# coecms/xmhw

Measured on AMD Instinct MI355X. Metric: grid-cells/sec for threshold() on 40yr daily SST, higher is better.
Workload: dtype f32 in / f64 out; 1 GPU; 0.25deg global (configs[2]): 1036800 cells per step, 1982-2021 (T=14610), windowHalfWidth=5, pctile=90, smoothPercentileWidth=31, nan_frac=0.0, skipna=False; cells_rank0=1036800, T=14610, D=366, kernel=clim_sorted_f32 (sorted row-lists in LDS, 2 lanes per cell, layout 40), slabs=1, gather=none

## Files before the change

include/xmhw_amd.h:

```cpp
#ifndef XMHW_AMD_H
#define XMHW_AMD_H

#include <stddef.h>
#include <stdint.h>

#ifdef __cplusplus
extern "C" {
#endif

#define XMHW_OK 0
#define XMHW_ERR_INVALID 1
#define XMHW_ERR_HIP 2
#define XMHW_ERR_UNSUPPORTED 3
#define XMHW_ERR_NOMEM 4
#define XMHW_ERR_COMM 5

#define XMHW_KERNEL_AUTO 0
#define XMHW_KERNEL_RING 1
#define XMHW_KERNEL_GENERIC 2

int xmhw_version(void);
const char *xmhw_arch(void);
const char *xmhw_last_error(void);
int xmhw_device_count(int *count);
// ... 29 lines not shown
                   void *dst_host);
int xmhw_pad_gaps(void *ts_dev, int itemsize, int64_t T, int64_t C, int64_t ld, const double *x_dev,
                  double max_gap, void *stream);
int xmhw_stream_create(void **stream);
int xmhw_stream_destroy(void *stream);
int xmhw_stream_sync(void *stream);
int xmhw_event_create(void **event);
int xmhw_stream_wait_event(void *stream, void *event);
int xmhw_event_destroy(void *event);
int xmhw_event_record(void *event, void *stream);
int xmhw_event_elapsed_ms(void *start, void *stop, float *ms);

typedef struct xmhw_plan xmhw_plan;

int xmhw_plan_create(const int32_t *doy_host, int64_t T, int32_t window_half_width,
                     xmhw_plan **plan);
int xmhw_plan_destroy(xmhw_plan *plan);
int xmhw_plan_info(const xmhw_plan *plan, int32_t *D, int32_t *ntracks,
                   int32_t *kernel, int32_t *nsteps, int32_t *step_min);
int xmhw_plan_doys(const xmhw_plan *plan, int32_t *doys_out );
int xmhw_plan_set_kernel(xmhw_plan *plan, int32_t kernel);
int xmhw_plan_set_narrowing(xmhw_plan *plan, int32_t enable);
int xmhw_plan_set_timing(xmhw_plan *plan, int32_t enable);
int xmhw_plan_kernel_ms(xmhw_plan *plan, int32_t calls_back, float *ms);
int xmhw_plan_narrowed(xmhw_plan *plan, int32_t *narrowed_out);
int xmhw_plan_set_chunks(xmhw_plan *plan, int32_t nchunks);
int xmhw_plan_chunks_in_use(const xmhw_plan *plan, int64_t C, int32_t *nchunks);
int xmhw_plan_table(const xmhw_plan *plan, int32_t years_per_lane, uint32_t *table_out,
                    int32_t *ntracks_padded);
int xmhw_plan_sorted_info(const xmhw_plan *plan, int64_t C, int32_t *keys_per_list, int32_t *lds_bytes_per_wave,
                          int32_t *pieces);
int xmhw_plan_sorted_table(const xmhw_plan *plan, int32_t pieces, int32_t *nchunks, int32_t *nrows, int32_t *ntp,
                           int32_t *chunks_out, uint32_t *table_out, uint32_t *flags_out);

int xmhw_debug_stats_available(void);
int xmhw_plan_debug_stats_n(xmhw_plan *plan, int enable, uint64_t *out, int32_t n);
int xmhw_plan_debug_stats(xmhw_plan *plan, int enable, uint64_t *out8);

enum {
    XMHW_LAYOUT_AUTO = -2,
    XMHW_LAYOUT_RING1 = -1,
    XMHW_LAYOUT_RING2_8LANE = 8,
    XMHW_LAYOUT_RING2_4LANE = 10,
    XMHW_LAYOUT_RING2_16LANE = 12,
    XMHW_LAYOUT_RING3_8LANE = 20,
    XMHW_LAYOUT_RING3_4LANE = 21,
    XMHW_LAYOUT_RING3_2LANE = 22,
    XMHW_LAYOUT_SORTED = 40
};
int xmhw_plan_set_layout(xmhw_plan *plan, int32_t layout);
int xmhw_plan_layout_in_use(const xmhw_plan *plan, int32_t *layout);
int xmhw_sorted_device_ok(int32_t *holds);
int xmhw_plan_set_ring2(xmhw_plan *plan, int32_t variant);
int xmhw_plan_ring2_in_use(const xmhw_plan *plan, int32_t *variant);
int xmhw_plan_f64_mode(const xmhw_plan *plan, int32_t *variant);

int xmhw_clim_raw_f32(xmhw_plan *plan, const float *ts_dev, int64_t C, int64_t ld,
                      double q, int negate, double *thresh_dev, double *seas_dev,
                      int64_t ldo, void *stream);
int xmhw_clim_raw_f64(xmhw_plan *plan, const double *ts_dev, int64_t C, int64_t ld,
                      double q, int negate, double *thresh_dev, double *seas_dev,
                      int64_t ldo, void *stream);
int xmhw_clim_raw_i16(xmhw_plan *plan, const int16_t *codes_dev, int64_t C, int64_t ld, int big_endian,
                      int has_scale, double scale_factor, double add_offset, int has_fill, int32_t fill_code,
                      int decoded_itemsize, double q, int negate, double *thresh_dev, double *seas_dev,
                      int64_t ldo, void *stream);
// ... 268 lines not shown
```

xmhw_amd/csrc/capi.cpp:

```cpp
#include "../../include/xmhw_amd.h"

#include <hip/hip_runtime.h>
#include <unistd.h>

#include <cerrno>
#include <cmath>

#include <algorithm>
#include <cstdio>
#include <cstdlib>
#include <atomic>
#include <cstring>
#include <map>
#include <memory>
#include <mutex>
#include <new>
#include <string>
#include <type_traits>
#include <vector>

#include "kernels.h"
#include "plan.h"

namespace {

thread_local std::string g_err;

int fail(int code, const std::string& msg) {
    g_err = msg;
    return code;
}
int hip_fail(hipError_t e, const char* what) {
    if (e == hipErrorOutOfMemory) {
        (void)hipGetLastError();
        return fail(XMHW_ERR_NOMEM, std::string(what) + ": out of device memory");
    }
    return fail(XMHW_ERR_HIP, std::string(what) + ": " + hipGetErrorString(e));
}
}
int xmhw_set_error_(int code, const std::string& msg) { return fail(code, msg); }
namespace {
#define HIP_TRY(expr)                                        \
    do {                                                     \
        hipError_t _e = (expr);                              \
        if (_e != hipSuccess) return hip_fail(_e, #expr);    \
    } while (0)

constexpr int kSubs = 8;
constexpr double kSortedMinQ = 0.85;
inline bool sorted_serves(double q) { return q >= kSortedMinQ || q <= 1.0 - kSortedMinQ; }

}

struct xmhw_plan {
    xmhw::Plan host;
    std::mutex mu;
    bool uploaded = false;
    int32_t yps = 0;
    int32_t subs = 0;
    int32_t nchunks = 0;
    uint32_t* d_table = nullptr;
    int32_t yps2 = 0;
    int32_t subs2 = 0;
    int32_t ring2_variant = -2;
    uint32_t* d_table2 = nullptr;
    uint32_t* d_sflags = nullptr;
    int32_t yps64 = 0;
    uint32_t* d_table64 = nullptr;
    xmhw::DevChunk* d_chunks = nullptr;
    int32_t* d_row_ptr = nullptr;
    int32_t* d_centres = nullptr;
    unsigned long long* d_stats = nullptr;
    uint32_t* d_tablex = nullptr;
    int32_t ypsx = 0, subsx = 0;
    uint32_t* d_narrow_flag = nullptr;
    bool narrowing = true;
    int32_t yps_s = 0;
    uint32_t* d_table_s = nullptr;
    xmhw::DevSortedChunk* d_chunks_s = nullptr;
    uint32_t* d_sflags_s = nullptr;
    xmhw::DevChunk* d_chunks_i = nullptr;
    int32_t nchunks_s = 0, nchunks_i = 0;
    int64_t sorted_pieces = -1;
    int32_t sorted_built = 0;
    bool timing = false;
    hipEvent_t tev[32] = {};
    uint64_t tcalls = 0;

    ~xmhw_plan() {
        if (d_stats) (void)hipFree(d_stats);
        for (hipEvent_t e : tev) if (e) (void)hipEventDestroy(e);
        if (d_table_s) (void)hipFree(d_table_s);
        if (d_chunks_s) (void)hipFree(d_chunks_s);
        if (d_sflags_s) (void)hipFree(d_sflags_s);
        if (d_chunks_i) (void)hipFree(d_chunks_i);
        if (d_narrow_flag) (void)hipFree(d_narrow_flag);
        if (d_tablex) (void)hipFree(d_tablex);
        if (d_table) (void)hipFree(d_table);
        if (d_table64) (void)hipFree(d_table64);
        if (d_table2) (void)hipFree(d_table2);
        if (d_sflags) (void)hipFree(d_sflags);
        if (d_chunks) (void)hipFree(d_chunks);
        if (d_row_ptr) (void)hipFree(d_row_ptr);
        if (d_centres) (void)hipFree(d_centres);
    }
};

namespace {

int32_t ring2_resolved(const xmhw_plan* p);
int32_t ring2_legacy(const xmhw_plan* p);

struct X64Choice { int32_t variant = -1, yps = 0; };
X64Choice x64_choice(const xmhw_plan* p) {
    static const bool on = [] { const char* v = std::getenv("XMHW_RING2_F64"); return !(v && v[0] == '0'); }();
    X64Choice c;
    if (!on || p->ring2_variant == -1) return c;
    const int32_t y8 = xmhw::ring2_pick_yps(p->host.w, p->host.ntracks, 8);
    static const bool lds_on = [] { const char* v = std::getenv("XMHW_RING2_F64_LDS"); return !(v && v[0] == '0'); }();
    static const bool r3_on = [] { const char* v = std::getenv("XMHW_RING3_F64"); return !(v && v[0] == '0'); }();
    static const bool r3_4 = [] { const char* v = std::getenv("XMHW_RING3_F64_LANES"); return !(v && v[0] == '8'); }();
    if (r3_on && r3_4) {
        const int32_t y4 = xmhw::ring3_pick_yps(p->host.w, p->host.ntracks, 4);
        if (y4 > 0 && xmhw::ring3_x64_supported(p->host.w, y4, 4)) {
            c.variant = 21;
            c.yps = y4;
            return c;
        }
    }
    if (r3_on && y8 > 0 && xmhw::ring3_pick_yps(p->host.w, p->host.ntracks, 8) == y8 &&
        xmhw::ring3_x64_supported(p->host.w, y8, 8)) {
        c.variant = 20;
        c.yps = y8;
        return c;
    }
    if (y8 > 0 && (y8 <= 4 || lds_on) && xmhw::ring2_x64_supported(p->host.w, y8, 8)) {
        c.variant = 8;
        c.yps = y8;
        return c;
    }
    const int32_t y16 = xmhw::ring2_pick_yps(p->host.w, p->host.ntracks, 12);
    if (y16 > 0 && y16 <= 6 && xmhw::ring2_x64_supported(p->host.w, y16, 12)) {
        c.variant = 12;
        c.yps = y16;
// ... 88 lines not shown
    static std::mutex mu;
    static int state[64];
    static bool init = false;
    std::lock_guard<std::mutex> lock(mu);
    if (!init) { for (int& v : state) v = -1; init = true; }
    int dev = 0;
    if (hipGetDevice(&dev) != hipSuccess || dev < 0 || dev >= 64) return 0;
    if (state[dev] >= 0) return state[dev];
    uint32_t* d_bad = nullptr;
    uint32_t bad = 1;
    if (hipMalloc(&d_bad, sizeof(uint32_t)) != hipSuccess) return 0;
    const bool ran = xmhw::sorted_lds_probe(d_bad, nullptr) == hipSuccess &&
                     hipMemcpy(&bad, d_bad, sizeof(uint32_t), hipMemcpyDeviceToHost) == hipSuccess;
    (void)hipFree(d_bad);
    if (!ran) return 0;
    state[dev] = bad == 0 ? 1 : 0;
    return state[dev];
}

int upload_sorted(xmhw_plan* p, int64_t C) {
    const xmhw::Plan& h = p->host;
    if (!sorted_usable(p) || sorted_device_ok() != 1) { p->nchunks_s = 0; return XMHW_OK; }
    const int32_t yps = xmhw::sorted_pick_yps(h.w, h.ntracks);
    const int64_t waves = (C + 31) / 32;
    const int64_t pieces = h.nchunks_req > 0 ? h.nchunks_req : (1536 + waves - 1) / std::max<int64_t>(waves, 1);
    if (!p->d_table_s || p->yps_s != yps || p->sorted_pieces != pieces) {
        HIP_TRY(hipDeviceSynchronize());
        for (void** q : {reinterpret_cast<void**>(&p->d_table_s), reinterpret_cast<void**>(&p->d_sflags_s),
                         reinterpret_cast<void**>(&p->d_chunks_s), reinterpret_cast<void**>(&p->d_chunks_i)})
            if (*q) { HIP_TRY(hipFree(*q)); *q = nullptr; }
        const xmhw::Plan::SortedPlan sp = h.sorted_plan(2 * yps, 24, pieces);
        p->sorted_built = 0;
        p->nchunks_i = 0;
        if (!sp.chunks.empty()) {
            std::vector<xmhw::DevSortedChunk> cs(sp.chunks.size());
            for (size_t i = 0; i < cs.size(); ++i) cs[i] = {sp.chunks[i].warm_start, sp.chunks[i].begin, sp.chunks[i].end, sp.chunks[i].trow0};
            std::stable_sort(cs.begin(), cs.end(), [](const xmhw::DevSortedChunk& a, const xmhw::DevSortedChunk& b) {
                return a.end - a.warm_start > b.end - b.warm_start;
            });
            HIP_TRY(hipMalloc(&p->d_table_s, sizeof(uint32_t) * sp.table.size()));
            HIP_TRY(hipMemcpy(p->d_table_s, sp.table.data(), sizeof(uint32_t) * sp.table.size(), hipMemcpyHostToDevice));
            HIP_TRY(hipMalloc(&p->d_sflags_s, sizeof(uint32_t) * sp.flags.size()));
            HIP_TRY(hipMemcpy(p->d_sflags_s, sp.flags.data(), sizeof(uint32_t) * sp.flags.size(), hipMemcpyHostToDevice));
            HIP_TRY(hipMalloc(&p->d_chunks_s, sizeof(xmhw::DevSortedChunk) * cs.size()));
            HIP_TRY(hipMemcpy(p->d_chunks_s, cs.data(), sizeof(xmhw::DevSortedChunk) * cs.size(), hipMemcpyHostToDevice));
            p->sorted_built = static_cast<int32_t>(cs.size());
        }
        p->yps_s = yps;
        p->sorted_pieces = pieces;
    }
    p->nchunks_s = p->sorted_built;
    return XMHW_OK;
}

int upload(xmhw_plan* p, int64_t C) {
    std::lock_guard<std::mutex> lock(p->mu);
    {
        const int rc = upload_sorted(p, C);
        if (rc != XMHW_OK) return rc;
    }
    const int32_t nchunks = auto_chunks(p, C);
    const X64Choice xc0 = x64_choice(p);
    const int32_t xsubs0 = xc0.variant == 21 ? 4 : 8;
    const bool need_x = (xc0.variant == 8 || xc0.variant == 20 || xc0.variant == 21) &&
                        !(p->subs2 == xsubs0 && p->yps2 == xc0.yps);
    if (p->uploaded && nchunks == p->nchunks &&
        p->subs2 == xmhw::ring2_subs(ring2_resolved(p)) &&
        p->yps2 == (ring2_resolved(p) >= 0 ? xmhw::ring2_pick_yps(p->host.w, p->host.ntracks, ring2_resolved(p)) : 0) &&
        (!need_x || (p->ypsx == xc0.yps && p->subsx == xsubs0)))
        return XMHW_OK;
    const xmhw::Plan& h = p->host;
    if (!p->uploaded) {
// ... 63 lines not shown
template <typename T>
int clim_raw(xmhw_plan* plan, const T* ts, int64_t C, int64_t ld, double q, int negate,
             double* thresh, double* seas, int64_t ldo, void* stream) {
    if (!plan) return fail(XMHW_ERR_INVALID, "plan is NULL");
    if (C < 0 || ld < C || ldo < C) return fail(XMHW_ERR_INVALID, "bad C/ld/ldo");
    if (!(q >= 0.0 && q <= 1.0)) return fail(XMHW_ERR_INVALID, "quantile must be in [0, 1]");
    if (C == 0) return XMHW_OK;
    if (!ts || !thresh || !seas) return fail(XMHW_ERR_INVALID, "NULL device buffer");
    const int32_t kernel = resolve_kernel(plan, sizeof(T));
    if (kernel < 0)
        return fail(XMHW_ERR_UNSUPPORTED, "ring kernel not available for this window/track count/dtype");
    int rc = upload(plan, C);
    if (rc != XMHW_OK) return rc;
    hipStream_t st = static_cast<hipStream_t>(stream);
    const xmhw::Plan& h = plan->host;
    hipError_t e;
    if (kernel == XMHW_KERNEL_RING) {
        if constexpr (sizeof(T) == 4) {
            const bool sorted = plan->nchunks_s > 0 && sorted_serves(q);
            const xmhw::DevChunk* rchunks = sorted ? plan->d_chunks_i : plan->d_chunks;
            const int32_t rn = sorted ? plan->nchunks_i : plan->nchunks;
            unsigned long long* rstats = sorted ? nullptr : plan->d_stats;
            e = hipSuccess;
            hipEvent_t t0 = nullptr, t1 = nullptr;
            if (plan->timing) {
                const int slot = static_cast<int>(plan->tcalls % 16);
                for (int i = 0; i < 2; ++i)
                    if (!plan->tev[2 * slot + i]) HIP_TRY(hipEventCreate(&plan->tev[2 * slot + i]));
                t0 = plan->tev[2 * slot];
                t1 = plan->tev[2 * slot + 1];
                plan->tcalls++;
            }
            if (sorted) {
                if (t0) e = hipEventRecord(t0, st);
                if (e == hipSuccess)
                    e = xmhw::launch_sorted_f32(reinterpret_cast<const float*>(ts), C, ld, h.T, plan->d_table_s,
                                                plan->d_sflags_s, plan->d_chunks_s, plan->nchunks_s, h.w,
                                                plan->yps_s, h.ntracks, q, negate, thresh, seas, ldo, st, plan->d_stats);
                if (e == hipSuccess && t1) e = hipEventRecord(t1, st);
            } else if (t0) {
                e = hipEventRecord(t0, st);
            }
            if (e != hipSuccess) {
            } else if (rn == 0) {
            } else
            if (plan->yps2 && ring2_resolved(plan) >= 0 && xmhw::ring2_f32_supported(h.w, plan->yps2, ring2_resolved(plan)))
                e = xmhw::launch_ring2_f32(reinterpret_cast<const float*>(ts), C, ld, h.T, plan->d_table2, plan->d_sflags,
                                           h.step_min, rchunks, rn, h.w, plan->yps2, h.ntracks,
                                           ring2_resolved(plan), q, negate, thresh, seas, ldo, st, rstats);
            else
            e = xmhw::launch_ring_f32(reinterpret_cast<const float*>(ts), C, ld, plan->d_table,
                                      h.step_min, rchunks, rn, h.w, plan->yps, plan->subs, q,
                                      negate, thresh, seas, ldo, st, rstats);
            if (e == hipSuccess && !sorted && t1) e = hipEventRecord(t1, st);
        } else {
            const uint32_t* run_flag = nullptr;
            e = hipSuccess;
            const NarrowChoice nc = narrow_choice(plan);
            if (plan->narrowing && nc.variant >= 0) {
                if (!plan->d_narrow_flag) HIP_TRY(hipMalloc(&plan->d_narrow_flag, sizeof(uint32_t)));
                e = xmhw::launch_narrow_probe(reinterpret_cast<const double*>(ts), h.T, C, ld, plan->d_narrow_flag, st);
                if (e == hipSuccess)
                    e = xmhw::launch_ring2_f32_narrowing(reinterpret_cast<const double*>(ts), C, ld, h.T, nc.table,
                                                         plan->d_sflags, h.step_min, plan->d_chunks, plan->nchunks, h.w,
                                                         nc.yps, h.ntracks, nc.variant, q, negate, thresh, seas, ldo, st,
                                                         plan->d_narrow_flag);
                run_flag = plan->d_narrow_flag;
            } else if (plan->narrowing && plan->yps) {
                if (!plan->d_narrow_flag) HIP_TRY(hipMalloc(&plan->d_narrow_flag, sizeof(uint32_t)));
                e = xmhw::launch_ring_f32_narrowing(reinterpret_cast<const double*>(ts), h.T, C, ld, plan->d_table,
                                                    h.step_min, plan->d_chunks, plan->nchunks, h.w, plan->yps,
                                                    plan->subs, q, negate, thresh, seas, ldo, st, plan->d_stats,
// ... 887 lines not shown
    return XMHW_OK;
}
int xmhw_plan_debug_stats(xmhw_plan* plan, int enable, uint64_t* out8) {
    return xmhw_plan_debug_stats_n(plan, enable, out8, 8);
}
int xmhw_plan_table(const xmhw_plan* plan, int32_t years_per_lane, uint32_t* table_out,
                    int32_t* ntracks_padded) {
    if (!plan) return fail(XMHW_ERR_INVALID, "plan is NULL");
    if (years_per_lane <= 0) return fail(XMHW_ERR_INVALID, "years_per_lane must be > 0");
    if (plan->host.ntracks > kSubs * years_per_lane)
        return fail(XMHW_ERR_INVALID, "years_per_lane too small for the number of tracks");
    if (ntracks_padded) *ntracks_padded = kSubs * years_per_lane;
    if (table_out) {
        std::vector<uint32_t> tab = plan->host.ring_table(kSubs, years_per_lane);
        std::memcpy(table_out, tab.data(), sizeof(uint32_t) * tab.size());
    }
    return XMHW_OK;
}

int xmhw_plan_sorted_info(const xmhw_plan* plan, int64_t C, int32_t* keys_per_list, int32_t* lds_bytes_per_wave,
                          int32_t* pieces) {
    if (!plan) return fail(XMHW_ERR_INVALID, "plan is NULL");
    const int32_t k = xmhw::sorted_pick_k(plan->host.w, plan->host.ntracks);
    if (k == 0) return fail(XMHW_ERR_UNSUPPORTED, "the sorted-list kernel is not instantiated for this window / record length");
    if (keys_per_list) *keys_per_list = k;
    if (lds_bytes_per_wave) *lds_bytes_per_wave = xmhw::sorted_lds_bytes(plan->host.w, plan->host.ntracks);
    if (pieces) {
        const int64_t waves = (std::max<int64_t>(C, 1) + 31) / 32;
        *pieces = static_cast<int32_t>(plan->host.nchunks_req > 0 ? plan->host.nchunks_req : (1536 + waves - 1) / waves);
    }
    return XMHW_OK;
}

int xmhw_plan_sorted_table(const xmhw_plan* plan, int32_t pieces, int32_t* nchunks, int32_t* nrows, int32_t* ntp,
                           int32_t* chunks_out, uint32_t* table_out, uint32_t* flags_out) {
    if (!plan) return fail(XMHW_ERR_INVALID, "plan is NULL");
    const int32_t yps = xmhw::sorted_pick_yps(plan->host.w, plan->host.ntracks);
    if (yps == 0) return fail(XMHW_ERR_UNSUPPORTED, "the sorted-list kernel is not instantiated for this window / record length");
    const xmhw::Plan::SortedPlan sp = plan->host.sorted_plan(2 * yps, 24, std::max(pieces, 1));
    if (nchunks) *nchunks = static_cast<int32_t>(sp.chunks.size());
    if (nrows) *nrows = static_cast<int32_t>(sp.flags.size());
    if (ntp) *ntp = 2 * yps;
    if (chunks_out)
        for (size_t i = 0; i < sp.chunks.size(); ++i) {
            chunks_out[4 * i + 0] = sp.chunks[i].warm_start;
            chunks_out[4 * i + 1] = sp.chunks[i].begin;
            chunks_out[4 * i + 2] = sp.chunks[i].end;
            chunks_out[4 * i + 3] = sp.chunks[i].trow0;
        }
    if (table_out) std::memcpy(table_out, sp.table.data(), sizeof(uint32_t) * sp.table.size());
    if (flags_out) std::memcpy(flags_out, sp.flags.data(), sizeof(uint32_t) * sp.flags.size());
    return XMHW_OK;
}

int xmhw_clim_raw_f32(xmhw_plan* plan, const float* ts, int64_t C, int64_t ld, double q, int negate,
                      double* thresh, double* seas, int64_t ldo, void* stream) {
    return clim_raw<float>(plan, ts, C, ld, q, negate, thresh, seas, ldo, stream);
}
int xmhw_clim_raw_f64(xmhw_plan* plan, const double* ts, int64_t C, int64_t ld, double q, int negate,
                      double* thresh, double* seas, int64_t ldo, void* stream) {
    return clim_raw<double>(plan, ts, C, ld, q, negate, thresh, seas, ldo, stream);
}

int xmhw_clim_raw_i16(xmhw_plan* plan, const int16_t* codes, int64_t C, int64_t ld, int big_endian, int has_scale,
                      double scale_factor, double add_offset, int has_fill, int32_t fill_code, int decoded_itemsize, double q,
                      int negate, double* thresh, double* seas, int64_t ldo, void* stream) {
// ... 10 lines not shown
    if (!(plan->nchunks_s > 0 && sorted_serves(q)))
        return fail(XMHW_ERR_UNSUPPORTED, "packed input runs on the sorted-list kernel only (w = 5, 9..48 tracks, quantile >= 0.85 or <= 0.15): "
                                         "decode the series (xmhw_decode) and call xmhw_clim_raw_f32 / _f64");
    xmhw::PackedI16 pk;
    pk.swap = big_endian ? 1 : 0;
    pk.fill = has_fill ? fill_code : 0x7FFFFFFF;
    int kneg = negate ? 1 : 0;
    if (!has_scale) {
        pk.mode = 3;
    } else if (decoded_itemsize == 4) {
        pk.mode = 1;
        pk.sf = static_cast<float>(scale_factor);
        pk.of = static_cast<float>(add_offset);
    } else {
        pk.mode = 2;
        pk.s = scale_factor;
        pk.o = add_offset;
        pk.val_neg = negate ? 1 : 0;
        kneg = (negate ? 1 : 0) ^ (scale_factor < 0.0 ? 1 : 0);
    }
    pk.key_neg = kneg;
    hipStream_t st = static_cast<hipStream_t>(stream);
    const xmhw::Plan& h = plan->host;
    hipEvent_t t0 = nullptr, t1 = nullptr;
    if (plan->timing) {
        const int slot = static_cast<int>(plan->tcalls % 16);
        for (int i = 0; i < 2; ++i)
            if (!plan->tev[2 * slot + i]) HIP_TRY(hipEventCreate(&plan->tev[2 * slot + i]));
        t0 = plan->tev[2 * slot];
        t1 = plan->tev[2 * slot + 1];
        plan->tcalls++;
    }
    hipError_t e = hipSuccess;
    if (t0) e = hipEventRecord(t0, st);
    if (e == hipSuccess)
        e = xmhw::launch_sorted_i16(codes, pk, C, ld, h.T, plan->d_table_s, plan->d_sflags_s, plan->d_chunks_s, plan->nchunks_s,
                                    h.w, plan->yps_s, h.ntracks, q, kneg, thresh, seas, ldo, st);
    if (e == hipSuccess && t1) e = hipEventRecord(t1, st);
    if (e != hipSuccess) return hip_fail(e, "packed climatology launch");
    return XMHW_OK;
}

int xmhw_clim_finish(const xmhw_plan* plan, const double* thresh_in, const double* seas_in, int64_t C,
                     int64_t ldo, int feb29_fix, int smooth, int smooth_width, double* thresh_out,
                     double* seas_out, void* stream) {
    if (!plan) return fail(XMHW_ERR_INVALID, "plan is NULL");
    if (smooth && (smooth_width <= 0 || smooth_width % 2 == 0))
        return fail(XMHW_ERR_INVALID, "Running average window should be odd");
    if (C < 0 || ldo < C) return fail(XMHW_ERR_INVALID, "bad C/ldo");
    if (C == 0) return XMHW_OK;
    if (!thresh_in || !seas_in || !thresh_out || !seas_out)
        return fail(XMHW_ERR_INVALID, "NULL device buffer");
    if (thresh_in == thresh_out || seas_in == seas_out)
        return fail(XMHW_ERR_INVALID, "in and out may not alias");
    const xmhw::Plan& h = plan->host;
    void* flags = nullptr;
    ScratchRef scratch_keep;
    if (smooth && smooth_width == 31) {
        hipError_t se = scratch_get(static_cast<hipStream_t>(stream), static_cast<size_t>(C), &flags, &scratch_keep);
        if (se != hipSuccess) return hip_fail(se, "scratch allocation");
    }
    hipError_t e = xmhw::launch_finish(thresh_in, seas_in, C, ldo, h.D, row_index(h, 59), row_index(h, 60),
                                       row_index(h, 61), feb29_fix, smooth, smooth ? smooth_width : 1,
                                       thresh_out, seas_out, static_cast<hipStream_t>(stream),
                                       static_cast<uint8_t*>(flags));
    if (e != hipSuccess) return hip_fail(e, "clim_finish launch");
    return XMHW_OK;
}

int xmhw_clim_f32(const float* ts, const int32_t* doy, int64_t T, int64_t C, int32_t D, int32_t w,
                  double q, int smooth, int smooth_w, int feb29_fix, int negate, double* thresh,
// ... 545 lines not shown
```

xmhw_amd/csrc/kernels.h:

```cpp
#pragma once
#include <hip/hip_runtime.h>
#include <stdint.h>

namespace xmhw {

struct DevChunk { int32_t warm_start, begin, end; };
struct PackedI16 {
    int32_t mode = 0;
    int32_t fill = 0x7FFFFFFF;
    int32_t swap = 0;
    int32_t key_neg = 0;
    int32_t val_neg = 0;
    float sf = 1.0f, of = 0.0f;
    double s = 1.0, o = 0.0;
};
struct DevSortedChunk { int32_t warm_start, begin, end, trow0; };

template <typename T>
hipError_t launch_generic(const T* ts, int64_t Tn, int64_t C, int64_t ld, const int32_t* row_ptr,
                          const int32_t* centres, int32_t D, int32_t w, double q, int negate,
                          double* thresh, double* seas, int64_t ldo, hipStream_t stream,
                          const uint32_t* run_flag = nullptr);

bool ring_supported(int32_t w, int32_t yps, int32_t subs, int elem_bytes);
// ... 16 lines not shown
bool ring2_x64_supported(int32_t w, int32_t yps, int32_t variant);
hipError_t launch_ring2_f64(const double* ts, int64_t C, int64_t ld, int64_t Tn, const uint32_t* table,
                            const uint32_t* sflags, int32_t step_min, const DevChunk* chunks, int32_t nchunks,
                            int32_t w, int32_t yps, int32_t ntracks, int32_t variant, double q, int negate,
                            double* thresh, double* seas, int64_t ldo, hipStream_t stream, const uint32_t* run_flag);
bool ring_stats_built();
int32_t ring2_subs(int32_t variant);
hipError_t launch_ring2_f32(const float* ts, int64_t C, int64_t ld, int64_t Tn, const uint32_t* table,
                            const uint32_t* sflags, int32_t step_min, const DevChunk* chunks, int32_t nchunks,
                            int32_t w, int32_t yps, int32_t ntracks, int32_t variant, double q, int negate,
                            double* thresh, double* seas, int64_t ldo, hipStream_t stream,
                            unsigned long long* stats = nullptr);

int32_t ring3_pick_yps(int32_t w, int32_t ntracks, int32_t subs);
bool ring3_supported(int32_t w, int32_t yps, int32_t subs);
hipError_t launch_ring3_f32(const float* ts, int64_t C, int64_t ld, int64_t Tn, const uint32_t* table,
                            const uint32_t* sflags, int32_t step_min, const DevChunk* chunks, int32_t nchunks,
                            int32_t w, int32_t yps, int32_t subs, int32_t ntracks, double q, int negate,
                            double* thresh, double* seas, int64_t ldo, hipStream_t stream,
                            unsigned long long* stats = nullptr);

int32_t sorted_pick_yps(int32_t w, int32_t ntracks);
int32_t sorted_pick_k(int32_t w, int32_t ntracks);
int32_t sorted_lds_bytes(int32_t w, int32_t ntracks);
hipError_t sorted_lds_probe(uint32_t* d_bad, hipStream_t stream);
hipError_t launch_sorted_f32(const float* ts, int64_t C, int64_t ld, int64_t Tn, const uint32_t* table,
                             const uint32_t* sflags, const DevSortedChunk* chunks, int32_t nchunks,
                             int32_t w, int32_t yps, int32_t ntracks, double q, int negate, double* thresh, double* seas,
                             int64_t ldo, hipStream_t stream, unsigned long long* stats = nullptr);
hipError_t launch_sorted_i16(const int16_t* codes, const PackedI16& pk, int64_t C, int64_t ld, int64_t Tn,
                             const uint32_t* table, const uint32_t* sflags, const DevSortedChunk* chunks, int32_t nchunks,
                             int32_t w, int32_t yps, int32_t ntracks, double q, int negate, double* thresh, double* seas,
                             int64_t ldo, hipStream_t stream);

int32_t ring4_pick_yps(int32_t w, int32_t ntracks, int32_t subs);
bool ring4_supported(int32_t w, int32_t yps, int32_t subs);
bool ring4_stats_built();
hipError_t launch_ring4_f32(const float* ts, int64_t C, int64_t ld, int64_t Tn, const uint32_t* table,
                            const uint32_t* sflags, int32_t step_min, const DevChunk* chunks, int32_t nchunks,
                            int32_t w, int32_t yps, int32_t subs, int32_t ntracks, double q, int negate,
                            double* thresh, double* seas, int64_t ldo, hipStream_t stream,
                            unsigned long long* stats = nullptr);

bool ring3_x64_supported(int32_t w, int32_t yps, int32_t subs);
hipError_t launch_ring3_f64(const double* ts, int64_t C, int64_t ld, int64_t Tn, const uint32_t* table,
                            const uint32_t* sflags, int32_t step_min, const DevChunk* chunks, int32_t nchunks,
                            int32_t w, int32_t yps, int32_t subs, int32_t ntracks, double q, int negate, double* thresh,
                            double* seas, int64_t ldo, hipStream_t stream, const uint32_t* run_flag);
bool ring3_narrowing_supported(int32_t w, int32_t yps, int32_t subs);
hipError_t launch_ring3_f32_narrowing(const double* ts, int64_t C, int64_t ld, int64_t Tn, const uint32_t* table,
                                      const uint32_t* sflags, int32_t step_min, const DevChunk* chunks,
                                      int32_t nchunks, int32_t w, int32_t yps, int32_t subs, int32_t ntracks, double q,
                                      int negate, double* thresh, double* seas, int64_t ldo, hipStream_t stream,
                                      uint32_t* narrow_flag);

hipError_t launch_ring_f32_narrowing(const double* ts, int64_t Tn, int64_t C, int64_t ld, const uint32_t* table,
                                     int32_t step_min, const DevChunk* chunks, int32_t nchunks, int32_t w,
                                     int32_t yps, int32_t subs, double q, int negate, double* thresh, double* seas,
                                     int64_t ldo, hipStream_t stream, unsigned long long* stats,
                                     uint32_t* narrow_flag);

hipError_t launch_finish(const double* th_in, const double* se_in, int64_t C, int64_t ldo, int32_t D,
                         int32_t i59, int32_t i60, int32_t i61, int feb29_fix, int smooth,
                         int32_t width, double* th_out, double* se_out, hipStream_t stream,
                         uint8_t* flags = nullptr);

// ... 190 lines not shown
```

xmhw_amd/csrc/plan.cpp:

```cpp
#include "plan.h"

#include <algorithm>

namespace xmhw {

bool Plan::build(const int32_t* doy, int64_t T_, int32_t w_) {
    if (T_ <= 0) { error = "time axis is empty"; return false; }
    if (w_ < 0) { error = "windowHalfWidth must be >= 0"; return false; }
    if (T_ > (int64_t(1) << 30) - 4) { error = "time axis too long"; return false; }
    T = T_;
    w = w_;
    R = 2 * w + 1;
    doys.assign(doy, doy + T);
    std::sort(doys.begin(), doys.end());
    doys.erase(std::unique(doys.begin(), doys.end()), doys.end());
    D = static_cast<int32_t>(doys.size());
    row_of_t.resize(T);
    for (int64_t t = 0; t < T; ++t)
        row_of_t[t] = static_cast<int32_t>(std::lower_bound(doys.begin(), doys.end(), doy[t]) - doys.begin());
    track_begin.clear();
    track_end.clear();
    track_begin.push_back(0);
    for (int64_t t = 1; t < T; ++t) {
        if (doy[t] <= doy[t - 1]) {
            track_end.push_back(t);
            track_begin.push_back(t);
        }
    }
    track_end.push_back(T);
    ntracks = static_cast<int32_t>(track_begin.size());
    row_ptr.assign(D + 1, 0);
    for (int64_t t = 0; t < T; ++t) row_ptr[row_of_t[t] + 1]++;
    max_centres = 0;
    for (int32_t r = 0; r < D; ++r) {
        max_centres = std::max(max_centres, row_ptr[r + 1]);
// ... 154 lines not shown
            ch.end = e;
            ch.trow0 = static_cast<int32_t>(out.flags.size());
            const int32_t nrows = e - ch.warm_start;
            const size_t base = out.table.size();
            out.table.resize(base + static_cast<size_t>(nrows) * ntp, make_entry(kCodeInvalid, true));
            for (int32_t k = 0; k < ntracks; ++k) {
                if (!inS[k]) continue;
                for (int32_t s = b; s < e; ++s)
                    out.table[base + static_cast<size_t>(s - ch.warm_start) * ntp + k] = orig(s, k);
                int32_t src = b;
                for (int32_t i = 1; i <= R - 1; ++i) {
                    uint32_t ent = make_entry(kCodeInvalid, true);
                    while (src > step_min) {
                        --src;
                        const uint32_t o = orig(src, k);
                        if ((o >> 1) != kCodeHold) { ent = o | 1u; break; }
                    }
                    out.table[base + static_cast<size_t>(b - i - ch.warm_start) * ntp + k] = ent;
                }
            }
            for (int32_t v = 0; v < nrows; ++v) {
                bool simple = true, consec = v > 0;
                for (int32_t k = 0; k < ntracks; ++k) {
                    const uint32_t en = out.table[base + static_cast<size_t>(v) * ntp + k];
                    simple = simple && (en >> 1) >= 2u;
                    if (v > 0) {
                        const uint32_t pr = out.table[base + static_cast<size_t>(v - 1) * ntp + k];
                        consec = consec && (en >> 1) >= 2u && (pr >> 1) >= 2u && (en >> 1) == (pr >> 1) + 1u;
                    }
                }
                out.flags.push_back((simple ? 1u : 0u) | (consec ? 2u : 0u));
            }
            out.chunks.push_back(ch);
        }
    }
    return out;
}

}
```

xmhw_amd/csrc/plan.h:

```cpp
#pragma once
#include <cstdint>
#include <string>
#include <vector>

namespace xmhw {

constexpr uint32_t kCodeHold = 0;
constexpr uint32_t kCodeInvalid = 1;
constexpr uint32_t make_entry(uint32_t code, bool counted) { return (code << 1) | (counted ? 1u : 0u); }

struct Chunk {
    int32_t warm_start;
    int32_t begin;
    int32_t end;
};

struct Plan {
    int64_t T = 0;
    int32_t w = 0;
    int32_t R = 1;
    int32_t D = 0;
    std::vector<int32_t> doys;
    std::vector<int32_t> row_of_t;
    int32_t ntracks = 0;
    std::vector<int64_t> track_begin, track_end;
    std::vector<int32_t> row_ptr;
    std::vector<int32_t> centres;
    int32_t max_centres = 0;
    int32_t step_min = 0;
    int32_t nsteps = 0;
    int32_t kernel_choice = 0;
    int32_t nchunks_req = 0;

    std::string error;

    bool build(const int32_t* doy, int64_t T, int32_t w);
    std::vector<uint32_t> ring_table(int32_t subs, int32_t yps) const;
    std::vector<uint32_t> step_flags() const;
    std::vector<Chunk> make_chunks(int32_t nchunks) const;
    int32_t warm_start_for(int32_t begin) const;
    struct Segment { int32_t begin, end; bool regular; };
    std::vector<Segment> sorted_segments() const;
    struct SortedChunk { int32_t warm_start, begin, end, trow0; };
    struct SortedPlan {
        std::vector<SortedChunk> chunks;
        std::vector<uint32_t> table, flags;
    };
    SortedPlan sorted_plan(int32_t ntp, int32_t min_rows_per_piece, int64_t pieces_wanted) const;
};

}
```

xmhw_amd/csrc/pybind.cpp:

```cpp
#include <pybind11/numpy.h>
#include <algorithm>
#include <pybind11/pybind11.h>

#include <cstdint>
#include <stdexcept>
#include <string>
#include <vector>

#include "../../include/xmhw_amd.h"

namespace py = pybind11;

namespace {

struct HipError : std::runtime_error { using std::runtime_error::runtime_error; };
struct Unsupported : HipError { using HipError::HipError; };
struct InvalidError : std::runtime_error { using std::runtime_error::runtime_error; };
struct CommError : std::runtime_error { using std::runtime_error::runtime_error; };

void check(int rc) {
    if (rc == XMHW_OK) return;
    std::string msg = xmhw_last_error();
    if (rc == XMHW_ERR_INVALID) throw InvalidError(msg);
    if (rc == XMHW_ERR_NOMEM) throw std::bad_alloc();
// ... 95 lines not shown
        py::array_t<int32_t> out(D);
        check(xmhw_plan_doys(pp(p), out.mutable_data()));
        return out;
    });
    m.def("plan_set_kernel", [](uintptr_t p, int k) { check(xmhw_plan_set_kernel(pp(p), k)); });
    m.def("plan_set_narrowing", [](uintptr_t p, int on) { check(xmhw_plan_set_narrowing(pp(p), on)); });
    m.def("plan_narrowed", [](uintptr_t p) { int32_t n = 0; check(xmhw_plan_narrowed(pp(p), &n)); return n != 0; });
    m.def("plan_set_chunks", [](uintptr_t p, int n) { check(xmhw_plan_set_chunks(pp(p), n)); });
    m.def("plan_table", [](uintptr_t p, int yps) {
        int32_t ns, ntp;
        check(xmhw_plan_info(pp(p), nullptr, nullptr, nullptr, &ns, nullptr));
        check(xmhw_plan_table(pp(p), yps, nullptr, &ntp));
        py::array_t<uint32_t> out({static_cast<py::ssize_t>(ns), static_cast<py::ssize_t>(ntp)});
        check(xmhw_plan_table(pp(p), yps, out.mutable_data(), &ntp));
        return out;
    });

    m.def("plan_set_timing", [](uintptr_t p, int on) { check(xmhw_plan_set_timing(pp(p), on)); });
    m.def("plan_kernel_ms", [](uintptr_t p, int back) { float ms = 0; check(xmhw_plan_kernel_ms(pp(p), back, &ms)); return ms; });
    m.def("plan_sorted_info", [](uintptr_t p, int64_t C) {
        int32_t k = 0, lds = 0, pieces = 0;
        check(xmhw_plan_sorted_info(pp(p), C, &k, &lds, &pieces));
        return py::make_tuple(k, lds, pieces);
    });
    m.def("plan_sorted_table", [](uintptr_t p, int pieces) {
        int32_t nc = 0, nr = 0, ntp = 0;
        check(xmhw_plan_sorted_table(pp(p), pieces, &nc, &nr, &ntp, nullptr, nullptr, nullptr));
        py::array_t<int32_t> chunks({static_cast<py::ssize_t>(nc), static_cast<py::ssize_t>(4)});
        py::array_t<uint32_t> table({static_cast<py::ssize_t>(nr), static_cast<py::ssize_t>(ntp)});
        py::array_t<uint32_t> flags(static_cast<py::ssize_t>(nr));
        check(xmhw_plan_sorted_table(pp(p), pieces, &nc, &nr, &ntp, chunks.mutable_data(), table.mutable_data(),
                                     flags.mutable_data()));
        return py::make_tuple(chunks, table, flags);
    });

    m.def("plan_debug_stats", [](uintptr_t p, int enable, bool read) {
        py::array_t<uint64_t> out(16);
        std::fill(out.mutable_data(), out.mutable_data() + 16, uint64_t(0));
        check(xmhw_plan_debug_stats_n(pp(p), enable, read ? out.mutable_data() : nullptr, 16));
        return out;
    });
    m.def("plan_chunks_in_use", [](uintptr_t p, int64_t C) { int32_t v = 0; check(xmhw_plan_chunks_in_use(pp(p), C, &v)); return v; });
    m.def("debug_stats_available", []() { return xmhw_debug_stats_available() != 0; });
    m.def("plan_set_layout", [](uintptr_t p, int layout) { check(xmhw_plan_set_layout(pp(p), layout)); });
    m.def("plan_layout_in_use", [](uintptr_t p) { int32_t v = -1; check(xmhw_plan_layout_in_use(pp(p), &v)); return v; });
    m.def("sorted_device_ok", []() { int32_t v = 0; check(xmhw_sorted_device_ok(&v)); return v != 0; });
    m.def("plan_ring2_in_use", [](uintptr_t p) { int32_t v = -1; check(xmhw_plan_ring2_in_use(pp(p), &v)); return v; });
    m.def("plan_f64_mode", [](uintptr_t p) { int32_t v = -1; check(xmhw_plan_f64_mode(pp(p), &v)); return v; });
    m.def("plan_set_ring2", [](uintptr_t p, int variant) { check(xmhw_plan_set_ring2(pp(p), variant)); });

    m.def("clim_raw", [](uintptr_t plan, uintptr_t ts, int itemsize, int64_t C, int64_t ld, double q, int negate,
                         uintptr_t th, uintptr_t se, int64_t ldo, uintptr_t stream) {
        if (itemsize == 4)
            check(xmhw_clim_raw_f32(pp(plan), static_cast<const float*>(vp(ts)), C, ld, q, negate,
                                    static_cast<double*>(vp(th)), static_cast<double*>(vp(se)), ldo, vp(stream)));
        else if (itemsize == 8)
            check(xmhw_clim_raw_f64(pp(plan), static_cast<const double*>(vp(ts)), C, ld, q, negate,
                                    static_cast<double*>(vp(th)), static_cast<double*>(vp(se)), ldo, vp(stream)));
        else throw InvalidError("itemsize must be 4 or 8");
    }, py::arg("plan"), py::arg("ts"), py::arg("itemsize"), py::arg("C"), py::arg("ld"), py::arg("q"),
       py::arg("negate"), py::arg("thresh"), py::arg("seas"), py::arg("ldo"), py::arg("stream") = 0);

    m.def("clim_raw_i16", [](uintptr_t plan, uintptr_t codes, int64_t C, int64_t ld, int big_endian, int has_scale,
                             double scale_factor, double add_offset, int has_fill, int32_t fill_code, int decoded_itemsize,
                             double q, int negate, uintptr_t th, uintptr_t se, int64_t ldo, uintptr_t stream) {
        check(xmhw_clim_raw_i16(pp(plan), static_cast<const int16_t*>(vp(codes)), C, ld, big_endian, has_scale, scale_factor,
// ... 587 lines not shown
```

xmhw_amd/device.py:

```python
import os as _os
import sys
import threading as _threading
import time as _time
from concurrent.futures import ThreadPoolExecutor
from contextlib import contextmanager

import numpy as np

from ._lib import hip
from .exception import XmhwException

KERNELS = {"auto": 0, "ring": 1, "generic": 2}


class PackedArray(np.ndarray):

    def __new__(cls, array, decode):
        obj = np.asarray(array).view(cls)
        obj.decode = dict(decode)
        return obj

    def __array_finalize__(self, obj):
        if obj is not None:
            self.decode = getattr(obj, "decode", None)
# ... 185 lines not shown
        self._h.plan_set_kernel(self.handle, KERNELS[kernel])
        self._h.plan_set_chunks(self.handle, int(nchunks))
        self._h.plan_set_narrowing(self.handle, int(bool(narrowing)))
        if layout is None:
            layout = ring2
        if layout is not None:
            self._h.plan_set_layout(self.handle, int(LAYOUTS.get(layout, layout)))
        info = self._h.plan_info(self.handle)
        self.D = info["D"]
        self.ntracks = info["ntracks"]
        self.kernel = {v: k for k, v in KERNELS.items()}.get(info["kernel"], "unsupported")
        self.nsteps = info["nsteps"]
        self.step_min = info["step_min"]
        self.doys = self._h.plan_doys(self.handle).astype(np.int64)
        self.T = doy.shape[0]
        self.w = int(window_half_width)

    def layout_in_use(self):
        return int(self._h.plan_layout_in_use(self.handle))

    ring2_in_use = layout_in_use

    def chunks_in_use(self, C):
        return int(self._h.plan_chunks_in_use(self.handle, int(C)))

    def f64_mode(self):
        return int(self._h.plan_f64_mode(self.handle))

    def narrowed(self):
        return bool(self._h.plan_narrowed(self.handle))

    def table(self, years_per_lane):
        return self._h.plan_table(self.handle, years_per_lane)

    def destroy(self):
        if getattr(self, "handle", 0):
            self._h.plan_destroy(self.handle)
            self.handle = 0

    def __del__(self):
        try:
            self.destroy()
        except Exception:
            pass


def clim_raw(plan, ts_dev, itemsize, C, q, negate, thresh_dev, seas_dev, ld=None, ldo=None, stream=0):
    with as_xmhw_errors():
        hip().clim_raw(plan.handle, _ptr(ts_dev), itemsize, C, C if ld is None else ld, float(q), int(bool(negate)),
                       _ptr(thresh_dev), _ptr(seas_dev), C if ldo is None else ldo, stream)


def clim_raw_packed(plan, codes_dev, C, q, negate, thresh_dev, seas_dev, scale_factor=None, add_offset=None, fill=None,
                    decoded="float32", big_endian=False, ld=None, ldo=None, stream=0):
    has_scale = scale_factor is not None or add_offset is not None
    with as_xmhw_errors(also="HipError"):
        hip().clim_raw_i16(plan.handle, _ptr(codes_dev), C, C if ld is None else ld, int(bool(big_endian)), int(has_scale),
                           1.0 if scale_factor is None else float(scale_factor), 0.0 if add_offset is None else float(add_offset),
                           int(fill is not None), 0 if fill is None else int(fill), 8 if str(decoded) in ("float64", "f64", "8") else 4,
                           float(q), int(bool(negate)), _ptr(thresh_dev), _ptr(seas_dev), C if ldo is None else ldo, stream)


def clim_finish(plan, th_in, se_in, C, feb29_fix, smooth, width, th_out, se_out, ldo=None, stream=0):
    with as_xmhw_errors():
        hip().clim_finish(plan.handle, _ptr(th_in), _ptr(se_in), C, C if ldo is None else ldo, int(bool(feb29_fix)),
                          int(bool(smooth)), int(width), _ptr(th_out), _ptr(se_out), stream)
# ... 510 lines not shown
```

Baseline: 42.74 million cells/s.

## Offload small single-row sorted chunks to a direct per-cell top-k kernel

Adds a second kernel that handles single-day sorted chunks with small sample pools (e.g. irregular days like Feb 29) by doing a per-thread register top-k over the gathered samples, instead of running them in the LDS sorted-list kernel. Chunks are reordered so these direct rows come last, the main sorted launch skips them, and a follow-up launch covers them. The aim is to stop these tail chunks from holding wave slots in the heavy LDS kernel. The cost is an extra launch, plus planning logic that must pick the right key count for the requested quantile.

```diff
diff --git a/include/xmhw_amd.h b/include/xmhw_amd.h
--- a/include/xmhw_amd.h
+++ b/include/xmhw_amd.h
@@ -85,6 +85,8 @@
                           int32_t *pieces);
 int xmhw_plan_sorted_table(const xmhw_plan *plan, int32_t pieces, int32_t *nchunks, int32_t *nrows, int32_t *ntp,
                            int32_t *chunks_out, uint32_t *table_out, uint32_t *flags_out);
+int xmhw_plan_set_direct_rows(xmhw_plan *plan, int32_t enable);
+int xmhw_plan_direct_info(const xmhw_plan *plan, double q, int32_t *rows, int32_t *keys, uint64_t *launches);
 
 int xmhw_debug_stats_available(void);
 int xmhw_plan_debug_stats_n(xmhw_plan *plan, int enable, uint64_t *out, int32_t n);
diff --git a/xmhw_amd/csrc/capi.cpp b/xmhw_amd/csrc/capi.cpp
--- a/xmhw_amd/csrc/capi.cpp
+++ b/xmhw_amd/csrc/capi.cpp
@@ -49,6 +49,21 @@
 constexpr int kSubs = 8;
 constexpr double kSortedMinQ = 0.85;
 inline bool sorted_serves(double q) { return q >= kSortedMinQ || q <= 1.0 - kSortedMinQ; }
+inline bool direct_rows_env() {
+    static const bool on = [] { const char* v = std::getenv("XMHW_DIRECT_ROWS"); return !(v && v[0] == '0'); }();
+    return on;
+}
+inline int32_t direct_tail(const std::vector<int32_t>& pools, double q, int32_t* keys) {
+    int32_t n = 0, k = 0;
+    for (size_t i = pools.size(); i-- > 0;) {
+        const int32_t ki = xmhw::direct_keys(pools[i], q);
+        if (ki == 0) break;
+        k = std::max(k, ki);
+        ++n;
+    }
+    if (keys) *keys = k;
+    return n;
+}
 
 }
 
@@ -83,6 +98,9 @@
     int32_t nchunks_s = 0, nchunks_i = 0;
     int64_t sorted_pieces = -1;
     int32_t sorted_built = 0;
+    std::vector<int32_t> direct_pool_s;
+    int32_t direct_rows = -1;
+    uint64_t direct_launches = 0;
     bool timing = false;
     hipEvent_t tev[32] = {};
     uint64_t tcalls = 0;
@@ -110,6 +128,11 @@
 
 int32_t ring2_resolved(const xmhw_plan* p);
 int32_t ring2_legacy(const xmhw_plan* p);
+constexpr int64_t kDirectMinCells = 8 * 2048 * 32;
+inline bool direct_rows_on(const xmhw_plan* p, int64_t C) {
+    if (p->direct_rows >= 0) return p->direct_rows != 0;
+    return direct_rows_env() && C >= kDirectMinCells;
+}
 
 struct X64Choice { int32_t variant = -1, yps = 0; };
 X64Choice x64_choice(const xmhw_plan* p) {
@@ -264,12 +287,23 @@
         const xmhw::Plan::SortedPlan sp = h.sorted_plan(2 * yps, 24, pieces);
         p->sorted_built = 0;
         p->nchunks_i = 0;
+        p->direct_pool_s.clear();
         if (!sp.chunks.empty()) {
+            std::vector<size_t> order(sp.chunks.size());
+            for (size_t i = 0; i < order.size(); ++i) order[i] = i;
+            std::stable_sort(order.begin(), order.end(), [&](size_t a, size_t b) {
+                const int32_t da = sp.direct_pool[a], db = sp.direct_pool[b];
+                if ((da != 0) != (db != 0)) return da == 0;
+                if (da != 0) return da > db;
+                return sp.chunks[a].end - sp.chunks[a].warm_start > sp.chunks[b].end - sp.chunks[b].warm_start;
+            });
             std::vector<xmhw::DevSortedChunk> cs(sp.chunks.size());
-            for (size_t i = 0; i < cs.size(); ++i) cs[i] = {sp.chunks[i].warm_start, sp.chunks[i].begin, sp.chunks[i].end, sp.chunks[i].trow0};
-            std::stable_sort(cs.begin(), cs.end(), [](const xmhw::DevSortedChunk& a, const xmhw::DevSortedChunk& b) {
-                return a.end - a.warm_start > b.end - b.warm_start;
-            });
+            p->direct_pool_s.clear();
+            for (size_t i = 0; i < cs.size(); ++i) {
+                const xmhw::Plan::SortedChunk& c = sp.chunks[order[i]];
+                cs[i] = {c.warm_start, c.begin, c.end, c.trow0};
+                if (sp.direct_pool[order[i]] != 0) p->direct_pool_s.push_back(sp.direct_pool[order[i]]);
+            }
             HIP_TRY(hipMalloc(&p->d_table_s, sizeof(uint32_t) * sp.table.size()));
             HIP_TRY(hipMemcpy(p->d_table_s, sp.table.data(), sizeof(uint32_t) * sp.table.size(), hipMemcpyHostToDevice));
             HIP_TRY(hipMalloc(&p->d_sflags_s, sizeof(uint32_t) * sp.flags.size()));
@@ -399,12 +433,20 @@
                 plan->tcalls++;
             }
             if (sorted) {
+                int32_t dkeys = 0;
+                const int32_t nd = direct_rows_on(plan, C) ? direct_tail(plan->direct_pool_s, q, &dkeys) : 0;
                 if (t0) e = hipEventRecord(t0, st);
                 if (e == hipSuccess)
                     e = xmhw::launch_sorted_f32(reinterpret_cast<const float*>(ts), C, ld, h.T, plan->d_table_s,
-                                                plan->d_sflags_s, plan->d_chunks_s, plan->nchunks_s, h.w,
+                                                plan->d_sflags_s, plan->d_chunks_s, plan->nchunks_s - nd, h.w,
                                                 plan->yps_s, h.ntracks, q, negate, thresh, seas, ldo, st, plan->d_stats);
                 if (e == hipSuccess && t1) e = hipEventRecord(t1, st);
+                if (e == hipSuccess && nd > 0) {
+                    e = xmhw::launch_direct_row_f32(reinterpret_cast<const float*>(ts), C, ld, h.T, plan->d_table_s,
+                                                    2 * plan->yps_s, plan->d_chunks_s + (plan->nchunks_s - nd), nd, dkeys, q,
+                                                    negate, thresh, seas, ldo, st);
+                    plan->direct_launches++;
+                }
             } else if (t0) {
                 e = hipEventRecord(t0, st);
             }
@@ -1358,6 +1400,31 @@
     return XMHW_OK;
 }
 
+int xmhw_plan_set_direct_rows(xmhw_plan* plan, int32_t enable) {
+    if (!plan) return fail(XMHW_ERR_INVALID, "plan is NULL");
+    plan->direct_rows = enable < 0 ? -1 : (enable != 0 ? 1 : 0);
+    return XMHW_OK;
+}
+
+int xmhw_plan_direct_info(const xmhw_plan* plan, double q, int32_t* rows, int32_t* keys, uint64_t* launches) {
+    if (!plan) return fail(XMHW_ERR_INVALID, "plan is NULL");
+    if (!(q >= 0.0 && q <= 1.0)) return fail(XMHW_ERR_INVALID, "quantile must be in [0, 1]");
+    int32_t nd = 0, k = 0;
+    const int32_t yps = xmhw::sorted_pick_yps(plan->host.w, plan->host.ntracks);
+    if (yps != 0 && sorted_usable(plan) && sorted_serves(q) && direct_rows_on(plan, kDirectMinCells)) {
+        const xmhw::Plan::SortedPlan sp = plan->host.sorted_plan(2 * yps, 24, 1);
+        std::vector<int32_t> pools;
+        for (int32_t v : sp.direct_pool)
+            if (v != 0) pools.push_back(v);
+        std::sort(pools.begin(), pools.end(), [](int32_t a, int32_t b) { return a > b; });
+        nd = direct_tail(pools, q, &k);
+    }
+    if (rows) *rows = nd;
+    if (keys) *keys = k;
+    if (launches) *launches = plan->direct_launches;
+    return XMHW_OK;
+}
+
 int xmhw_plan_sorted_table(const xmhw_plan* plan, int32_t pieces, int32_t* nchunks, int32_t* nrows, int32_t* ntp,
                            int32_t* chunks_out, uint32_t* table_out, uint32_t* flags_out) {
     if (!plan) return fail(XMHW_ERR_INVALID, "plan is NULL");
@@ -1434,11 +1501,18 @@
         plan->tcalls++;
     }
     hipError_t e = hipSuccess;
+    int32_t dkeys = 0;
+    const int32_t nd = direct_rows_on(plan, C) ? direct_tail(plan->direct_pool_s, q, &dkeys) : 0;
     if (t0) e = hipEventRecord(t0, st);
     if (e == hipSuccess)
-        e = xmhw::launch_sorted_i16(codes, pk, C, ld, h.T, plan->d_table_s, plan->d_sflags_s, plan->d_chunks_s, plan->nchunks_s,
-                                    h.w, plan->yps_s, h.ntracks, q, kneg, thresh, seas, ldo, st);
+        e = xmhw::launch_sorted_i16(codes, pk, C, ld, h.T, plan->d_table_s, plan->d_sflags_s, plan->d_chunks_s,
+                                    plan->nchunks_s - nd, h.w, plan->yps_s, h.ntracks, q, kneg, thresh, seas, ldo, st);
     if (e == hipSuccess && t1) e = hipEventRecord(t1, st);
+    if (e == hipSuccess && nd > 0) {
+        e = xmhw::launch_direct_row_i16(codes, pk, C, ld, h.T, plan->d_table_s, 2 * plan->yps_s,
+                                        plan->d_chunks_s + (plan->nchunks_s - nd), nd, dkeys, q, kneg, thresh, seas, ldo, st);
+        plan->direct_launches++;
+    }
     if (e != hipSuccess) return hip_fail(e, "packed climatology launch");
     return XMHW_OK;
 }
diff --git a/xmhw_amd/csrc/kernels.h b/xmhw_amd/csrc/kernels.h
--- a/xmhw_amd/csrc/kernels.h
+++ b/xmhw_amd/csrc/kernels.h
@@ -72,6 +72,14 @@
                              const uint32_t* table, const uint32_t* sflags, const DevSortedChunk* chunks, int32_t nchunks,
                              int32_t w, int32_t yps, int32_t ntracks, double q, int negate, double* thresh, double* seas,
                              int64_t ldo, hipStream_t stream);
+
+hipError_t launch_direct_row_f32(const float* ts, int64_t C, int64_t ld, int64_t Tn, const uint32_t* table, int32_t ntp,
+                                 const DevSortedChunk* chunks, int32_t nchunks, int32_t keys, double q, int negate,
+                                 double* thresh, double* seas, int64_t ldo, hipStream_t stream);
+hipError_t launch_direct_row_i16(const int16_t* codes, const PackedI16& pk, int64_t C, int64_t ld, int64_t Tn,
+                                 const uint32_t* table, int32_t ntp, const DevSortedChunk* chunks, int32_t nchunks,
+                                 int32_t keys, double q, int negate, double* thresh, double* seas, int64_t ldo,
+                                 hipStream_t stream);
 
 int32_t ring4_pick_yps(int32_t w, int32_t ntracks, int32_t subs);
 bool ring4_supported(int32_t w, int32_t yps, int32_t subs);
diff --git a/xmhw_amd/csrc/kernels_direct_row.hip b/xmhw_amd/csrc/kernels_direct_row.hip
--- /dev/null
+++ b/xmhw_amd/csrc/kernels_direct_row.hip
@@ -0,0 +1,172 @@
+#include <type_traits>
+
+#include "device_common.h"
+#include "kernels.h"
+#include "packed_src.h"
+#include "plan.h"
+
+namespace xmhw {
+namespace {
+
+constexpr int kDirectBlock = 256;
+constexpr int kDirectGroup = 16;
+constexpr int kDirectR = 11;
+
+__device__ __forceinline__ uint32_t dmed3u(uint32_t a, uint32_t b, uint32_t c) {
+    uint32_t r;
+    asm("v_med3_u32 %0, %1, %2, %3" : "=v"(r) : "v"(a), "v"(b), "v"(c));
+    return r;
+}
+__device__ __forceinline__ uint32_t dumin(uint32_t a, uint32_t b) { return a < b ? a : b; }
+__device__ __forceinline__ uint32_t dumax(uint32_t a, uint32_t b) { return a > b ? a : b; }
+
+template <int M>
+__device__ __forceinline__ void top_insert(uint32_t (&top)[M], uint32_t key) {
+#pragma unroll
+    for (int i = M - 1; i >= 1; --i) top[i] = dmed3u(top[i - 1], top[i], key);
+    top[0] = dumax(top[0], key);
+}
+template <int M>
+__device__ __forceinline__ uint32_t top_pick(const uint32_t (&top)[M], uint32_t idx) {
+    uint32_t r = 0;
+#pragma unroll
+    for (int i = 0; i < M; ++i) r = idx == static_cast<uint32_t>(i) ? top[i] : r;
+    return r;
+}
+
+template <typename SRC, int M>
+__global__ __launch_bounds__(kDirectBlock) void clim_direct_row(
+    SRC src, int64_t C, int64_t ld, int64_t Tn, const uint32_t* __restrict__ table, int32_t ntp,
+    const DevSortedChunk* __restrict__ chunks, double q, int negate, double* __restrict__ thresh,
+    double* __restrict__ seas, int64_t ldo) {
+    using Raw = typename std::remove_cv<typename std::remove_reference<decltype(*src.p)>::type>::type;
+    constexpr int R = kDirectR;
+    const int64_t cell = static_cast<int64_t>(blockIdx.x) * kDirectBlock + threadIdx.x;
+    if (cell >= C) return;
+    const DevSortedChunk ch = chunks[blockIdx.y];
+    const bool mirror = q < 0.5;
+    const bool kneg = (negate != 0) != mirror;
+    const uint32_t tmax = static_cast<uint32_t>(Tn - 1);
+    const Raw* col = src.p + cell;
+    const uint32_t* rows = table + static_cast<int64_t>(ch.trow0) * ntp;
+    const int m0 = ((ch.warm_start % R) + R) % R;
+
+    uint32_t top[M];
+#pragma unroll
+    for (int i = 0; i < M; ++i) top[i] = 0u;
+    uint32_t n = 0;
+    double tsum0 = 0.0, tsum1 = 0.0;
+    for (int g = 0; g < R; ++g) {
+        const int v = g >= m0 ? g - m0 : g - m0 + R;
+        const uint32_t* row = rows + static_cast<int64_t>(v) * ntp;
+        double d0 = 0.0, d1 = 0.0;
+        for (int k0 = 0; k0 < ntp; k0 += kDirectGroup) {
+            uint32_t code[kDirectGroup];
+            Raw raw[kDirectGroup];
+#pragma unroll
+            for (int i = 0; i < kDirectGroup; ++i) code[i] = k0 + i < ntp ? row[k0 + i] >> 1 : kCodeInvalid;
+#pragma unroll
+            for (int i = 0; i < kDirectGroup; ++i) {
+                raw[i] = Raw(0);
+                if (code[i] >= 2u) raw[i] = col[static_cast<int64_t>(dumin(code[i] - 2u, tmax)) * ld];
+            }
+#pragma unroll
+            for (int i = 0; i < kDirectGroup; ++i) {
+                if (code[i] >= 2u) {
+                    float xs;
+                    if constexpr (std::is_same<Raw, int16_t>::value) xs = packed_sample(src.pk, packed_code(src.pk, raw[i]));
+                    else xs = raw[i];
+                    const bool ok = xs == xs;
+                    const uint32_t key = ok ? f32_key(kneg ? -xs : xs) : 0u;
+                    const double dv = static_cast<double>(ok ? xs : 0.0f);
+                    if (i & 1) d1 += dv;
+                    else d0 += dv;
+                    n += ok ? 1u : 0u;
+                    top_insert<M>(top, key);
+                }
+            }
+        }
+        if (negate) {
+            d0 = -d0;
+            d1 = -d1;
+        }
+        const double lsum = d0 + d1;
+        if (g < 6) tsum0 += lsum;
+        else tsum1 += lsum;
+    }
+    tsum1 += 0.0;
+    const double total = tsum0 + tsum1;
+
+    double th = make_nan(), se = make_nan();
+    if (n > 0) {
+        const double vi = static_cast<double>(n - 1u) * q;
+        const double fl = floor(vi);
+        const double gw = vi - fl;
+        const uint32_t lo = static_cast<uint32_t>(fl);
+        const bool need2 = lo + 1u < n;
+        uint32_t i_lo, i_hi;
+        if (mirror) {
+            i_lo = lo;
+            i_hi = need2 ? lo + 1u : lo;
+        } else {
+            i_lo = n - 1u - lo;
+            i_hi = need2 ? n - 2u - lo : i_lo;
+        }
+        double v_lo = static_cast<double>(key_f32(top_pick<M>(top, i_lo)));
+        double v_hi = static_cast<double>(key_f32(top_pick<M>(top, i_hi)));
+        if (mirror) {
+            v_lo = -v_lo;
+            v_hi = -v_hi;
+        }
+        se = total / static_cast<double>(n);
+        if constexpr (std::is_same<Raw, int16_t>::value) {
+            v_lo = packed_value(src.pk, v_lo);
+            v_hi = packed_value(src.pk, v_hi);
+            se = packed_value(src.pk, se);
+        }
+        th = numpy_lerp(v_lo, v_hi, gw);
+    }
+    const int64_t o = static_cast<int64_t>(ch.begin) * ldo + cell;
+    thresh[o] = th;
+    seas[o] = se;
+}
+
+template <typename SRC>
+hipError_t launch_direct(const SRC& src, int64_t C, int64_t ld, int64_t Tn, const uint32_t* table, int32_t ntp,
+                         const DevSortedChunk* chunks, int32_t nchunks, int32_t keys, double q, int negate, double* thresh,
+                         double* seas, int64_t ldo, hipStream_t stream) {
+    if (keys < 1 || keys > kDirectMaxKeys || ntp <= 0) return hipErrorInvalidValue;
+    if (C <= 0 || nchunks <= 0) return hipSuccess;
+    const dim3 grid(static_cast<unsigned>((C + kDirectBlock - 1) / kDirectBlock), static_cast<unsigned>(nchunks));
+    const dim3 block(kDirectBlock);
+    if (keys <= 12)
+        hipLaunchKernelGGL((clim_direct_row<SRC, 12>), grid, block, 0, stream, src, C, ld, Tn, table, ntp, chunks, q, negate,
+                           thresh, seas, ldo);
+    else if (keys <= 16)
+        hipLaunchKernelGGL((clim_direct_row<SRC, 16>), grid, block, 0, stream, src, C, ld, Tn, table, ntp, chunks, q, negate,
+                           thresh, seas, ldo);
+    else
+        hipLaunchKernelGGL((clim_direct_row<SRC, 24>), grid, block, 0, stream, src, C, ld, Tn, table, ntp, chunks, q, negate,
+                           thresh, seas, ldo);
+    return hipGetLastError();
+}
+
+}
+
+hipError_t launch_direct_row_f32(const float* ts, int64_t C, int64_t ld, int64_t Tn, const uint32_t* table, int32_t ntp,
+                                 const DevSortedChunk* chunks, int32_t nchunks, int32_t keys, double q, int negate,
+                                 double* thresh, double* seas, int64_t ldo, hipStream_t stream) {
+    return launch_direct(PlainSrc<float>{ts}, C, ld, Tn, table, ntp, chunks, nchunks, keys, q, negate, thresh, seas, ldo,
+                         stream);
+}
+
+hipError_t launch_direct_row_i16(const int16_t* codes, const PackedI16& pk, int64_t C, int64_t ld, int64_t Tn,
+                                 const uint32_t* table, int32_t ntp, const DevSortedChunk* chunks, int32_t nchunks,
+                                 int32_t keys, double q, int negate, double* thresh, double* seas, int64_t ldo,
+                                 hipStream_t stream) {
+    if (pk.mode < 1 || pk.mode > 3) return hipErrorInvalidValue;
+    return launch_direct(PackedSrc{codes, pk}, C, ld, Tn, table, ntp, chunks, nchunks, keys, q, negate, thresh, seas, ldo,
+                         stream);
+}
+
+}
diff --git a/xmhw_amd/csrc/plan.cpp b/xmhw_amd/csrc/plan.cpp
--- a/xmhw_amd/csrc/plan.cpp
+++ b/xmhw_amd/csrc/plan.cpp
@@ -1,6 +1,7 @@
 #include "plan.h"
 
 #include <algorithm>
+#include <cmath>
 
 namespace xmhw {
 
@@ -221,9 +222,29 @@
                 out.flags.push_back((simple ? 1u : 0u) | (consec ? 2u : 0u));
             }
             out.chunks.push_back(ch);
+            int32_t pool = 0;
+            bool any_simple = false;
+            for (int32_t v = 0; v < nrows; ++v) {
+                any_simple = any_simple || (out.flags[static_cast<size_t>(ch.trow0 + v)] & 1u) != 0;
+                for (int32_t k = 0; k < ntp; ++k)
+                    pool += (out.table[base + static_cast<size_t>(v) * ntp + k] >> 1) >= 2u ? 1 : 0;
+            }
+            const bool direct = e - b == 1 && !any_simple && pool >= 1 && pool <= kDirectMaxPool;
+            out.direct_pool.push_back(direct ? pool : 0);
         }
     }
     return out;
 }
 
-}
+int32_t direct_keys(int32_t pool_max, double q) {
+    if (pool_max < 1 || pool_max > kDirectMaxPool || !(q >= 0.0 && q <= 1.0)) return 0;
+    const bool mirror = q < 0.5;
+    int32_t need = 1;
+    for (int32_t n = 1; n <= pool_max; ++n) {
+        const int32_t lo = static_cast<int32_t>(std::floor(static_cast<double>(n - 1) * q));
+        need = std::max(need, mirror ? std::min(lo + 2, n) : n - lo);
+    }
+    return need <= kDirectMaxKeys ? need : 0;
+}
+
+}
diff --git a/xmhw_amd/csrc/plan.h b/xmhw_amd/csrc/plan.h
--- a/xmhw_amd/csrc/plan.h
+++ b/xmhw_amd/csrc/plan.h
@@ -45,8 +45,13 @@
     struct SortedPlan {
         std::vector<SortedChunk> chunks;
         std::vector<uint32_t> table, flags;
+        std::vector<int32_t> direct_pool;
     };
     SortedPlan sorted_plan(int32_t ntp, int32_t min_rows_per_piece, int64_t pieces_wanted) const;
 };
 
+constexpr int32_t kDirectMaxPool = 128;
+constexpr int32_t kDirectMaxKeys = 24;
+int32_t direct_keys(int32_t pool_max, double q);
+
 }
diff --git a/xmhw_amd/csrc/pybind.cpp b/xmhw_amd/csrc/pybind.cpp
--- a/xmhw_amd/csrc/pybind.cpp
+++ b/xmhw_amd/csrc/pybind.cpp
@@ -151,6 +151,14 @@
         check(xmhw_plan_sorted_table(pp(p), pieces, &nc, &nr, &ntp, chunks.mutable_data(), table.mutable_data(),
                                      flags.mutable_data()));
         return py::make_tuple(chunks, table, flags);
+    });
+
+    m.def("plan_set_direct_rows", [](uintptr_t p, int on) { check(xmhw_plan_set_direct_rows(pp(p), on)); });
+    m.def("plan_direct_info", [](uintptr_t p, double q) {
+        int32_t rows = 0, keys = 0;
+        uint64_t launches = 0;
+        check(xmhw_plan_direct_info(pp(p), q, &rows, &keys, &launches));
+        return py::make_tuple(rows, keys, launches);
     });
 
     m.def("plan_debug_stats", [](uintptr_t p, int enable, bool read) {
diff --git a/xmhw_amd/device.py b/xmhw_amd/device.py
--- a/xmhw_amd/device.py
+++ b/xmhw_amd/device.py
@@ -241,6 +241,13 @@
 
     def table(self, years_per_lane):
         return self._h.plan_table(self.handle, years_per_lane)
+
+    def set_direct_rows(self, enable):
+        self._h.plan_set_direct_rows(self.handle, -1 if enable is None else int(bool(enable)))
+
+    def direct_info(self, q):
+        rows, keys, launches = self._h.plan_direct_info(self.handle, float(q))
+        return int(rows), int(keys), int(launches)
 
     def destroy(self):
         if getattr(self, "handle", 0):
```

Result: no change. 42.68 million cells/s (-0.1%).
